# Yelp/nrtsearch

Hardware: AMD Instinct MI355X
Metric: queries/sec, 10M-doc 5-term BM25 top-1000 (higher is better)
Workload: dtype f32

## Files before the change

### nrtsearch_amd/csrc/maxscore.hip

```cpp
#include <hip/hip_runtime.h>
#include <stdint.h>

#include "bm25_common.hiph"

namespace nrtgpu {

constexpr int kMsWinWords = kMsWinDocs / 32;
constexpr int kSl = kMsSlots;
typedef uint32_t u32x2 __attribute__((ext_vector_type(2)));
typedef const NRT_GLOBAL u32x2* gvec2_ptr;

struct alignas(16) WClause {
  uint64_t docids, fnorm;
  uint64_t begin;
  uint32_t count, pad0;
  float    weight;
  int32_t  fx_scale;
  uint32_t flags;
  uint32_t pad;
  uint64_t u_after;
  uint64_t look;
  uint64_t cells, start;
};
static_assert(sizeof(WClause) == 80, "WClause layout");

struct MsSmem {
  uint64_t cand[kMsCandCap];
  uint32_t tab[kTabTerms][kTabEntries];
  float    cache[kLdsCaches][256];
  uint32_t seen[kMsWaves][kMsWinWords];
  WClause  wc[kMsWaves][kMsMaxTerms];
  TopkScratch sc;
  uint64_t theta;
  uint64_t thr;
// ... 175 lines not shown
        __hip_atomic_store(&s.theta, guess, __ATOMIC_RELAXED, __HIP_MEMORY_SCOPE_WORKGROUP);
        __hip_atomic_store(&s.thr, acc_threshold<true>(guess, fx_E), __ATOMIC_RELAXED, __HIP_MEMORY_SCOPE_WORKGROUP);
        atomicMax(theta_g, (unsigned long long)guess);
        atomicMax(s.spec_slot, (unsigned long long)guess);
      }
      s.spec_at = ws >= s.q_wins ? 0u : max(ws * s.spec_grow16 / 16u, ws + (uint32_t)kMsWaves);
      s.n_est += 1u;
    }
  }
  wave_lds_phase();
  if (lane == 0u) __hip_atomic_store(&s.spec_busy, 0u, __ATOMIC_RELEASE, __HIP_MEMORY_SCOPE_WORKGROUP);
}

__device__ __forceinline__ bool ms_reserve(MsSmem& s, uint32_t lane, uint32_t mine, uint32_t& pos) {
  const uint32_t incl = scan64_dpp(mine);
  const uint32_t wave_total = (uint32_t)__builtin_amdgcn_readlane((int)incl, 63);
  uint32_t wbase = 0;
  if (lane == 0) {
    wbase = atomicAdd(&s.cnt, wave_total);
    if (wbase + wave_total > (uint32_t)kMsCandCap) {
      if (wbase <= (uint32_t)kMsCandCap) s.cnt_valid = wbase;
      __hip_atomic_store(&s.rz_flag, 1u, __ATOMIC_RELAXED, __HIP_MEMORY_SCOPE_WORKGROUP);
    }
  }
  wbase = (uint32_t)__builtin_amdgcn_readfirstlane((int)wbase);
  pos = wbase + incl - mine;
  return wbase + wave_total <= (uint32_t)kMsCandCap;
}

template <bool PROF, bool PACKED, int SHAPES>
__global__ __launch_bounds__(kMsThreads)
void bm25_maxscore_kernel(const MsArgs* __restrict__ launch) {
  constexpr bool TWO = SHAPES == 2;
  __shared__ MsSmem s;
  const uint32_t tid = threadIdx.x;
  const uint32_t wave = tid >> 6, lane = tid & 63u;
  for (uint32_t round = 0;; ++round) {
    const uint64_t wall_entry = PROF ? wall_clock64() : 0ull;
    const ms_args_ptr ap = ms_fresh(launch);
    const __attribute__((address_space(4))) DHelp& hp = ap->help;
    const DItem* const items = as_global(ap->items);
    const DPart* const parts = as_global(ap->parts);
    const DWalkRow* const rows = as_global(ap->rows);
  #ifdef NRTGPU_DEV
    const DTerm* const terms = as_global(ap->terms);
  #endif
    const DExchange* const xch = as_global(ap->xch);
    bool helper = false;
    uint32_t my_item = 0, out_slot = 0;
    {
      const uint32_t min_rem = hp.min_rem & 0xFFFFu;
      const bool greedy = ((hp.min_rem >> 16) & 1u) != 0u;
      for (int attempt = 0; attempt < 2; ++attempt) {
        if (tid == 0) {
          s.pick = 0ull;
          s.role[0] = __hip_atomic_load(hp.item_next, __ATOMIC_RELAXED, __HIP_MEMORY_SCOPE_AGENT);
          s.role[1] = __hip_atomic_load(hp.help_used, __ATOMIC_RELAXED, __HIP_MEMORY_SCOPE_AGENT);
          s.role[2] = 0u;
          s.role[3] = __hip_atomic_load(hp.help_off, __ATOMIC_RELAXED, __HIP_MEMORY_SCOPE_AGENT);
        }
        __syncthreads();
        const uint32_t q_next = s.role[0];
        const bool queue_empty = attempt == 1 || q_next >= hp.n_own;
        const bool slots_left = s.role[1] < hp.n_help;
        if (queue_empty && (!slots_left || s.role[3] != 0u)) return;
        const bool look = slots_left && (queue_empty || (hp.alpha16 != 0u && q_next >= hp.n_cus + hp.n_cus / 4u));
// ... 83 lines not shown
    const float tie_breaker = TWO ? q.tie_breaker : 0.0f;
    auto loosen = [&](uint64_t t) { return (TWO && sec_mode == kMsSecReqOpt) ? max(t - (t >> 21), (uint64_t)2) - (uint64_t)1 : t; };
    unsigned int* const my_prune_g = as_global(ap->q_prune) + item.query;
    const uint64_t after_key = q.has_after ? pack_key(q.after_score, (uint32_t)q.after_doc) : ~0ull;

    {
      const uint32_t n_lds = min(item.n_caches, (uint32_t)kLdsCaches) * 256u;
      const float* const caches = as_global(ap->caches);
      for (uint32_t i = tid; i < n_lds; i += kMsThreads) (&s.cache[0][0])[i] = caches[item.cache_off + i];
    }
    for (uint32_t i = tid; i < (uint32_t)kMsCandCap; i += kMsThreads) s.cand[i] = 0ull;
    if (tid == 0) {
      const uint64_t theta0 = __hip_atomic_load(my_theta_g, __ATOMIC_RELAXED, __HIP_MEMORY_SCOPE_AGENT);
      s.theta = theta0;
      s.thr = acc_threshold<true>(theta0, fx_E);
      s.cnt = 0;
      s.cnt_valid = 0;
      s.rz_flag = 0;
      s.spec_busy = 0;
      s.n_meet = s.n_over = s.n_est = 0;
      if (!helper) {
        const unsigned long long now0 = (unsigned long long)wall_clock64();
        __hip_atomic_store(hp.item_t0 + my_item, now0, __ATOMIC_RELAXED, __HIP_MEMORY_SCOPE_AGENT);
        if (my_item == 0u) __hip_atomic_store(hp.t_start, now0, __ATOMIC_RELAXED, __HIP_MEMORY_SCOPE_AGENT);
      }
      s.prune_on = mode == kMsModePrune ? 1u : 0u;
      const bool spec = hp.spec_g != nullptr && hp.spec_z16 != 0u;
      s.wins_started = 0;
      s.q_wins = spec ? as_global(ap->q_wins)[item.query] : 0u;
      s.spec_z16 = spec ? hp.spec_z16 : 0u;
      s.spec_slot = spec ? as_global(hp.spec_g) + item.query : nullptr;
      s.spec_at = spec ? max(hp.spec_sched & 255u, 1u) : 0u;
      s.spec_grow16 = max((hp.spec_sched >> 8) & 255u, 17u);
      s.spec_meet = (hp.spec_sched >> 16) & 1u;
      for (int i = 0; i < kSliceSlots; ++i) s.slot_hits[i] = s.slot_slice[i] = 0u;
      for (int i = 0; i < 16; ++i) s.prof[i] = 0;
    }
    const uint64_t t_item0 = PROF ? __builtin_readcyclecounter() : 0ull;
    const uint64_t wall0 = PROF ? wall_clock64() : 0ull;
    uint64_t tc_meet = 0, tc_part = 0, tc_walk = 0;
    __syncthreads();
    if (xch && tid < 64u) {
      const uint64_t pb = exchange_bound(*xch, item.query, 0ull, tid);
      if (tid == 0 && pb > s.theta) {
        s.theta = pb;
        s.thr = acc_threshold<true>(pb, fx_E);
      }
    }
    for (uint32_t slot = 0; slot < item.n_tabs; ++slot) {
      const float w = items[my_item].tab_weight[slot];
      const int scale = items[my_item].tab_scale[slot];
      const float* cache = &s.cache[items[my_item].tab_cache[slot]][0];
      for (uint32_t e = tid; e < (uint32_t)kTabEntries; e += kMsThreads)
        s.tab[slot][e] = e < (uint32_t)kTabNorms ? 0u : score_value<true>(bm25_score(w, (float)(int32_t)(e >> 7), cache[e & 127u]), scale);
    }
    __syncthreads();
  #ifndef NRT_MS_PHASE_CLOCKS
    if (PROF && tid == 0) s.prof[8] = __builtin_readcyclecounter() - t_item0;
  #endif

    uint32_t* const seen = &s.seen[wave][0];
    WClause* const wcl = &s.wc[wave][0];
    const uint32_t wcl_addr = lds_addr(wcl);
    uint32_t wave_hits = 0;
    uint32_t cur_slot = 0;
    uint64_t pc_post = 0, pc_surv = 0, pc_look = 0, pc_cand = 0, pc_chunks = 0, pc_wins = 0;
  #ifdef NRT_MS_PHASE_CLOCKS
    uint64_t ph[9] = {0, 0, 0, 0, 0, 0, 0, 0, 0}, ph_t = 0;
  #endif
  #ifdef NRT_MS_COUNT_ROUNDS
    uint64_t pc_dense = 0, pc_sparse = 0, pc_steps = 0, pc_tas = 0, pc_crounds = 0;
  #endif
    const uint32_t item_wins = item.flags >> 8;
    uint32_t sc_mul = 1u;
    if (ap->scatter != 0u && item_wins > 3u && item_wins < 65536u) {
      const uint32_t primes[4] = {2654435761u, 2246822519u, 3266489917u, 668265263u};
      uint32_t best = 0xFFFFFFFFu;
  #pragma unroll
      for (int i = 0; i < 4; ++i) {
        const uint32_t a = primes[i] % item_wins;
        const uint32_t x = a * 1000u, y = item_wins * 618u;
        const uint32_t dist = x > y ? x - y : y - x;
        if (a > 1u && dist < best) {
          best = dist;
          sc_mul = a;
        }
      }
    }
    auto window_of_take = [&](uint32_t h) -> uint32_t {
      return (sc_mul == 1u || h >= item_wins) ? h : (h * sc_mul) % item_wins;
    };
    uint32_t g = window_of_take(helper ? (uint32_t)kMsWaves + (uint32_t)__builtin_amdgcn_readfirstlane((int)first_win) : wave);
    uint32_t pi = 0;
    uint32_t win_base = 0;

    const bool parts_by_lane = item.n_parts <= 64u;
    uint32_t part_incl = 0;
    if (parts_by_lane) {
      uint32_t w = 0;
      if (lane < item.n_parts) {
        const u32x2 tr = *(gvec2_ptr)&parts[item.part_begin + lane].tile_begin;
        w = (tr[1] - (tr[0] & ~(win_tiles - 1u)) + win_tiles - 1u) / win_tiles;
      }
      part_incl = scan64_dpp(w);
// ... 105 lines not shown
  #endif
      {
        static_assert(sizeof(DWalkRow) == sizeof(WClause) && sizeof(WClause) % 16 == 0, "a walk row is the image of a WClause");
        const gvec_ptr src = (gvec_ptr)(rows + part.term_begin);
        if (lane < n_terms * (uint32_t)(sizeof(WClause) / 16)) *(u32x4*)lds_ptr(wcl_addr + lane * 16u) = src[lane];
        wave_lds_phase();
        if (lane < n_terms) {
          const uint32_t rec = wcl_addr + lane * (uint32_t)sizeof(WClause);
          my_suf = *(const uint64_t*)lds_ptr(rec + 16u);
          my_flags = *(const uint32_t*)lds_ptr(rec + 40u);
          const u32x4 cs = *(const u32x4*)lds_ptr(rec + 64u);
          my_cells = (gu32_ptr)(((uint64_t)cs[1] << 32) | cs[0]);
          my_start = ((uint64_t)cs[3] << 32) | cs[2];
        }
        my_shift = (my_flags >> 16) & 31u;
      }
      const uint32_t req_mask = TWO ? (uint32_t)__builtin_amdgcn_ballot_w64(lane < n_terms && (my_flags & 8u) != 0u) : 0u;
      const uint32_t first_req = req_mask != 0u ? (uint32_t)__builtin_ctz(req_mask) : 0xFFu;
      if (PROF) tc_part += __builtin_readcyclecounter() - t_part0;

      for (;;) {
        const uint64_t t_win0 = PROF ? __builtin_readcyclecounter() : 0ull;
        const uint32_t ta = (part.tile_begin & ~(win_tiles - 1u)) + (g - win_base) * win_tiles;
        const uint32_t t0 = max(ta, part.tile_begin);
        const uint32_t t1 = min(ta + win_tiles, part.tile_end);
        const uint32_t doc_lo = t0 * (uint32_t)kTileDocs;
        const uint32_t doc_span = min(t1 * (uint32_t)kTileDocs, part.max_doc) - doc_lo;
        if (PROF) pc_wins += 1;
        {
          uint32_t est = 0;
          if (lane == 0) {
            const uint32_t ws = atomicAdd(&s.wins_started, 1u) + 1u, at = s.spec_at;
            if (at != 0u && ws >= at) {
              if (s.spec_meet != 0u) __hip_atomic_store(&s.rz_flag, 1u, __ATOMIC_RELAXED, __HIP_MEMORY_SCOPE_WORKGROUP);
              else est = atomicCAS(&s.spec_busy, 0u, 1u) == 0u ? 1u : 0u;
            }
          }
          if (__builtin_amdgcn_readfirstlane((int)est) != 0)
            ms_estimate((__attribute__((address_space(3))) MsSmem*)&s, k, fx_E, my_theta_g, xch);
        }
        uint32_t g_new = 0;
        if (lane == 0) g_new = (uint32_t)kMsWaves + __hip_atomic_fetch_add(win_next_g, 1u, __ATOMIC_RELAXED, __HIP_MEMORY_SCOPE_AGENT);
        uint64_t theta_other = 0, thr_other = 0;
        if (multi_item) {
          theta_other = __hip_atomic_load(my_theta_g, __ATOMIC_RELAXED, __HIP_MEMORY_SCOPE_AGENT);
          thr_other = acc_threshold<true>(theta_other, fx_E);
          if (mode == kMsModeCount && lane == 0 && __hip_atomic_load(my_prune_g, __ATOMIC_RELAXED, __HIP_MEMORY_SCOPE_AGENT) != 0u)
            __hip_atomic_store(&s.prune_on, 1u, __ATOMIC_RELAXED, __HIP_MEMORY_SCOPE_WORKGROUP);
        }
        uint32_t my_lo = 0, my_hi = 0;
        if (lane < n_terms) {
          my_lo = my_cells[t0 >> my_shift];
          my_hi = my_cells[((t1 - 1u) >> my_shift) + 1u];
        }
        if (n_terms > 1u) {
  #pragma unroll
          for (int j = 0; j < kMsWinWords / 64 / 4; ++j) *(u32x4*)&seen[(lane + 64u * (uint32_t)j) * 4u] = u32x4{0u, 0u, 0u, 0u};
        }
        uint32_t ng = 0;
        {
          const uint64_t thr_w = __hip_atomic_load(&s.prune_on, __ATOMIC_RELAXED, __HIP_MEMORY_SCOPE_WORKGROUP) ? loosen(max(s.thr, thr_other)) : 0ull;
          const uint64_t pb = my_start + my_lo, pe = my_start + my_hi;
          if (lane < n_terms) {
            if (my_suf >= thr_w && pe > pb && (!SHAPES || msm <= 1u || lane + msm <= n_terms) && (!TWO || lane <= first_req)) ng = (uint32_t)((pe - (pb & ~3ull) + (uint64_t)(kSl - 1)) / (uint64_t)kSl);
            *(u32x4*)&wcl[lane].begin = u32x4{(uint32_t)pb, (uint32_t)(pb >> 32), (uint32_t)(pe - pb), 0u};
          }
        }
        const uint32_t incl = scan32_dpp(ng);
        uint32_t pre[kMsMaxTerms];
  #pragma unroll
        for (int i = 0; i < kMsMaxTerms; ++i) pre[i] = (uint32_t)__builtin_amdgcn_readlane((int)incl, i);
        const uint32_t n_groups = pre[kMsMaxTerms - 1];

  #ifdef NRT_MS_PHASE_CLOCKS
        if (PROF) ph_t = t_win0;
  #endif
        NRT_PH_MARK(0);
        for (uint32_t v0 = 0; v0 < n_groups; v0 += 64u) {
          const uint32_t v = v0 + lane;
          const bool act = v < n_groups;
          uint32_t c = 0, before = 0;
  #pragma unroll
          for (int i = 0; i < kMsMaxTerms - 1; ++i) {
            c += (v >= pre[i]) ? 1u : 0u;
            before = (v >= pre[i]) ? pre[i] : before;
          }
          const uint32_t c_first = (uint32_t)__builtin_amdgcn_readfirstlane((int)c);
          const uint64_t theta = max(s.theta, theta_other), thr = loosen(max(s.thr, thr_other));
          const bool pruning = __hip_atomic_load(&s.prune_on, __ATOMIC_RELAXED, __HIP_MEMORY_SCOPE_WORKGROUP) != 0u;
          const uint64_t thr_p = pruning ? thr : 0ull;
          if (readlane_u64(my_suf, c_first) < thr_p) break;
          if (PROF) pc_chunks += 1;
          const uint32_t rec = wcl_addr + c * (uint32_t)sizeof(WClause);
          const u32x4 r0 = *(const u32x4*)lds_ptr(rec), r1 = *(const u32x4*)lds_ptr(rec + 16u), r2 = *(const u32x4*)lds_ptr(rec + 32u);
          const uint64_t u_after = *(const uint64_t*)lds_ptr(rec + 48u);
          const uint64_t col_d = ((uint64_t)r0[1] << 32) | r0[0], col_c = ((uint64_t)r0[3] << 32) | r0[2];
          const uint64_t p_begin = ((uint64_t)r1[1] << 32) | r1[0];
          const uint32_t flags = r2[2];
          const uint32_t q0 = (v - before) * (uint32_t)kSl;
          const uint64_t mine0 = (p_begin & ~3ull) + (uint64_t)q0;
          uint32_t d[kSl], cd[kSl];
  #pragma unroll
          for (int j = 0; j < kSl; ++j) d[j] = cd[j] = 0u;
          if (act) {
            const u32x4 d0 = __builtin_nontemporal_load((gvec_ptr)(col_d + mine0 * 4u));
            const u32x4 d1 = kSl > 4 ? __builtin_nontemporal_load((gvec_ptr)(col_d + mine0 * 4u) + 1) : d0;
            if (PACKED) {
              const uint32_t sw = doc_lo & ~kPackDocMask;
  #pragma unroll
              for (int j = 0; j < 4; ++j) {
                d[j] = (d0[j] >> kPackCodeBits) | sw;
                cd[j] = (d0[j] & kPackCodeMask) << 2;
                if (kSl > 4) {
                  d[(4 + j) % kSl] = (d1[j] >> kPackCodeBits) | sw;
                  cd[(4 + j) % kSl] = (d1[j] & kPackCodeMask) << 2;
                }
              }
            } else {
              const u32x4 c0 = __builtin_nontemporal_load((gvec_ptr)(col_c + mine0 * 4u));
              const u32x4 c1 = kSl > 4 ? __builtin_nontemporal_load((gvec_ptr)(col_c + mine0 * 4u) + 1) : c0;
  #pragma unroll
              for (int j = 0; j < 4; ++j) {
                d[j] = d0[j];
                cd[j] = c0[j];
                if (kSl > 4) {
                  d[(4 + j) % kSl] = d1[j];
                  cd[(4 + j) % kSl] = c1[j];
                }
              }
            }
          }
          NRT_PH_MARK(1);
          uint32_t vmask = 0;
          {
            const uint32_t rel = q0 - ((uint32_t)p_begin & 3u), cnt = act ? r1[2] : 0u;
  #pragma unroll
            for (int j = 0; j < kSl; ++j)
              if (rel + (uint32_t)j < cnt && d[j] - doc_lo < doc_span) vmask |= 1u << j;
          }
          uint32_t val[kSl];
          {
            const uint32_t tab = flags & 7u;
            const char* tb = (const char*)&s.tab[tab == 7u ? 0u : tab][0];
            uint32_t cor = 0;
  #pragma unroll
            for (int j = 0; j < kSl; ++j) {
              val[j] = *(const uint32_t*)(tb + (cd[j] & 0x1FFCu));
              const uint32_t cn = ((vmask >> j) & 1u) ? cd[j] : 0u;
              cor = PACKED ? max(cor, cn) : (cor | cn);
            }
            const bool special = vmask != 0u && ((PACKED ? cor >= (kPackEscBase << 2) : (cor >> 31) != 0u) || tab == 7u);
            if (__any(special)) {
              const float w = __uint_as_float(r2[0]);
              const int fx_scale = (int)r2[1];
              const float* cache = &s.cache[(flags >> 8) & 255u][0];
  #pragma unroll
              for (int j = 0; j < kSl; ++j) {
                uint32_t cj = cd[j];
                if (PACKED && cj >= (kPackEscBase << 2))
                  cj = ((vmask >> j) & 1u) ? packed_escape_word((gu32_ptr)col_c, (uint32_t)mine0 + (uint32_t)j, cj >> 2) : 0x80000100u;
                const bool esc = (cj >> 31) != 0u;
                const uint32_t f = esc ? ((cj >> 8) & 0x3FFFFFu) : ((cj >> 9) & 15u);
                const bool dead = esc ? ((cj >> 30) & 1u) != 0u : (cj >> 20) != 0u;
                const uint32_t nb = esc ? (cj & 255u) : ((cj >> 2) & 127u);
                if (((vmask >> j) & 1u) && (esc || tab == 7u))
                  val[j] = dead ? 0u : score_value<true>(bm25_score(w, (float)(int32_t)f, cache[nb]), fx_scale);
              }
            }
          }
          uint64_t run[kSl];
          uint32_t alive = 0;
          {
            const uint32_t mult = 1u << ((flags >> 4) & 15u);
            uint32_t need_v = 1u;
            if (u_after < thr_p) {
              const uint64_t gap = use_max ? thr_p : thr_p - u_after;
              const uint64_t nv = (gap + (uint64_t)(mult - 1u)) >> ((flags >> 4) & 15u);
              need_v = nv > 0xFFFFFFFFull ? 0xFFFFFFFFu : max((uint32_t)nv, 1u);
            }
            uint32_t pass = 0;
  #pragma unroll
            for (int j = 0; j < kSl; ++j) {
              run[j] = (uint64_t)val[j] * (uint64_t)mult;
              pass |= val[j] >= need_v ? (1u << j) : 0u;
            }
            alive = vmask & pass;
            if (need_v == 0xFFFFFFFFu) {
  #pragma unroll
              for (int j = 0; j < kSl; ++j)
                if ((use_max ? max(run[j], u_after) : run[j] + u_after) < thr_p) alive &= ~(1u << j);
            }
          }
          uint64_t sec[TWO ? kSl : 1];
          if (TWO) {
            if ((req_mask & ((1u << c) - 1u)) != 0u) alive = 0u;
            const bool mine_counts = sec_mode == kMsSecTieBreaker || (sec_mode == kMsSecReqOpt && ((req_mask >> c) & 1u) == 0u);
  #pragma unroll
            for (int j = 0; j < kSl; ++j) sec[j] = mine_counts ? run[j] : 0ull;
          }
          if (PROF) {
            pc_post += (uint64_t)__popc(vmask);
            pc_surv += (uint64_t)__popc(alive);
          }
          NRT_PH_MARK(2);
          const uint32_t c_last = (uint32_t)__builtin_amdgcn_readlane((int)c, (int)(min(n_groups - v0, 64u) - 1u));
          if (n_terms > 1u && __any(alive != 0u)) {
            for (uint32_t cc = c_first; cc <= c_last; ++cc) {
              const uint32_t am = c == cc ? alive : 0u;
              if (!__any(am != 0u)) continue;
  #ifdef NRT_MS_COUNT_ROUNDS
              if (PROF) pc_tas += 1;
  #endif
              uint32_t old[kSl];
  #pragma unroll
              for (int j = 0; j < kSl; ++j) {
                const bool a = (am >> j) & 1u;
                const uint32_t w = a ? ((d[j] - doc_lo) >> 5) : lane;
                old[j] = atomicOr(&seen[w], a ? (1u << (d[j] & 31u)) : 0u);
              }
  #pragma unroll
              for (int j = 0; j < kSl; ++j)
                if (((am >> j) & 1u) && ((old[j] >> (d[j] & 31u)) & 1u)) alive &= ~(1u << j);
            }
          }
          NRT_PH_MARK(3);
          uint32_t ccnt = 0x11111111u;

          for (uint32_t j2 = c_first + 1u; j2 < n_terms; ++j2) {
            if (!__any(alive != 0u)) break;
            const uint64_t S_j = readlane_u64(my_suf, j2);
            uint32_t am = c < j2 ? alive : 0u;
            {
              const uint64_t short_of = S_j < thr_p ? (use_max ? thr_p : thr_p - S_j) : 0ull;
              uint32_t kill = 0;
  #pragma unroll
              for (int j = 0; j < kSl; ++j) kill |= run[j] < short_of ? (1u << j) : 0u;
              if (SHAPES && msm > 1u) {
                const uint32_t left = n_terms - j2;
  #pragma unroll
                for (int j = 0; j < kSl; ++j) kill |= ((ccnt >> (4 * j)) & 15u) + left < msm ? (1u << j) : 0u;
              }
              kill &= am;
              alive &= ~kill;
              am &= ~kill;
            }
            if (!__any(am != 0u)) continue;
            if (PROF) pc_look += (uint64_t)__popc(am);
            const WClause& w2 = wcl[j2];
            const uint64_t look2 = uniform_u64(w2.look);
            const uint32_t flags2 = (uint32_t)__builtin_amdgcn_readfirstlane((int)w2.flags);
            const uint32_t kind2 = (flags2 >> 24) & 7u;
            const uint64_t start2 = uniform_u64(w2.start);
            const gu32_ptr codes2 = (gu32_ptr)(uniform_u64(PACKED ? w2.docids : w2.fnorm) + start2 * 4u);
            uint32_t c2[kSl];
            uint32_t pi2[kSl];
            uint32_t present = 0;
  #ifdef NRT_MS_COUNT_ROUNDS
            if (PROF) { if (kind2 == kLookBits) pc_dense += 1; else pc_sparse += 1; }
  #endif
            if (kind2 == kLookBits) {
              const gvec2_ptr recs = (gvec2_ptr)look2;
              u32x2 r[kSl];
  #pragma unroll
              for (int j = 0; j < kSl; ++j) r[j] = recs[((am >> j) & 1u) ? (d[j] >> 5) : 0u];
              __builtin_amdgcn_sched_barrier(0);
              NRT_PH_MARK(4);
              uint32_t idx[kSl];
  #pragma unroll
              for (int j = 0; j < kSl; ++j) {
                const uint32_t bb = d[j] & 31u;
                const bool there = ((am >> j) & 1u) && ((r[j][0] >> bb) & 1u);
                idx[j] = there ? r[j][1] + (uint32_t)__popc(r[j][0] & ((1u << bb) - 1u)) : 0u;
                present |= (there ? 1u : 0u) << j;
              }
  #pragma unroll
              for (int j = 0; j < kSl; ++j) c2[j] = codes2[idx[j]];
              __builtin_amdgcn_sched_barrier(0);
              NRT_PH_MARK(5);
  #pragma unroll
              for (int j = 0; j < kSl; ++j) pi2[j] = (uint32_t)start2 + idx[j];
            } else {
              const gu32_ptr cells2 = (gu32_ptr)(kind2 == kLookCells ? look2 : uniform_u64(w2.cells));
              const gu32_ptr docs2 = (gu32_ptr)(uniform_u64(w2.docids) + start2 * 4u);
              const uint32_t cshift = kind2 == kLookCells ? (flags2 >> 27) & 31u : 10u + ((flags2 >> 16) & 31u);
              uint32_t a[kSl], b[kSl];
  #pragma unroll
              for (int j = 0; j < kSl; ++j) {
                const uint32_t cell = ((am >> j) & 1u) ? (d[j] >> cshift) : 0u;
                a[j] = cells2[cell];
                b[j] = cells2[cell + 1u];
              }
              uint32_t open = 0;
  #pragma unroll
              for (int j = 0; j < kSl; ++j) {
                if (!((am >> j) & 1u)) b[j] = a[j];
                open |= (a[j] < b[j] ? 1u : 0u) << j;
              }
              while (__any(open != 0u)) {
  #ifdef NRT_MS_COUNT_ROUNDS
                if (PROF) pc_steps += 1;
  #endif
                uint32_t mid[kSl], vv[kSl];
  #pragma unroll
                for (int j = 0; j < kSl; ++j) {
                  mid[j] = (a[j] + b[j]) >> 1;
                  vv[j] = docs2[((open >> j) & 1u) ? mid[j] : 0u];
                }
  #pragma unroll
                for (int j = 0; j < kSl; ++j)
                  if ((open >> j) & 1u) {
                    const uint32_t dv = PACKED ? vv[j] >> kPackCodeBits : vv[j], dd = PACKED ? d[j] & kPackDocMask : d[j];
                    if (dv < dd) a[j] = mid[j] + 1u;
                    else b[j] = mid[j];
                    if (dv == dd) {
                      a[j] = b[j] = mid[j];
                      present |= 1u << j;
                    }
                    if (!(a[j] < b[j])) open &= ~(1u << j);
                  }
              }
  #pragma unroll
              for (int j = 0; j < kSl; ++j) {
                c2[j] = codes2[((present >> j) & 1u) ? a[j] : 0u];
                pi2[j] = (uint32_t)start2 + a[j];
              }
              NRT_PH_MARK(7);
            }
            if (__any(present != 0u)) {
              uint32_t v2[kSl];
              if (PACKED) {
  #pragma unroll
                for (int j = 0; j < kSl; ++j) c2[j] = (c2[j] & kPackCodeMask) << 2;
              }
              values_of_codes<PACKED, kSl>(s, c2, present, flags2 & 7u, w2.weight, w2.fx_scale, (flags2 >> 8) & 255u, w2.fnorm, pi2, v2);
              const uint32_t mult2 = 1u << ((flags2 >> 4) & 15u);
              if (use_max) {
  #pragma unroll
                for (int j = 0; j < kSl; ++j) run[j] = max(run[j], (uint64_t)(((present >> j) & 1u) ? v2[j] : 0u) * (uint64_t)mult2);
              } else if (TWO && sec_mode != kMsSecNone) {
                const bool counts = sec_mode == kMsSecReqOpt && (flags2 & 8u) == 0u;
  #pragma unroll
                for (int j = 0; j < kSl; ++j) {
                  const uint64_t add = (uint64_t)(((present >> j) & 1u) ? v2[j] : 0u) * (uint64_t)mult2;
                  run[j] += add;
                  sec[j] = sec_mode == kMsSecTieBreaker ? max(sec[j], add) : sec[j] + (counts ? add : 0ull);
                }
              } else {
  #pragma unroll
                for (int j = 0; j < kSl; ++j) run[j] += (uint64_t)(((present >> j) & 1u) ? v2[j] : 0u) * (uint64_t)mult2;
              }
              if (SHAPES && msm > 1u) {
                uint32_t x = present;
                x = (x | (x << 12)) & 0x000F000Fu;
                x = (x | (x << 6)) & 0x03030303u;
                x = (x | (x << 3)) & 0x11111111u;
                ccnt += x;
              }
            }
            if (TWO && (flags2 & 8u) != 0u) alive &= ~(am & ~present);
            NRT_PH_MARK(6);
          }

          {
          uint32_t maybe = 0;
  #pragma unroll
          for (int j = 0; j < kSl; ++j)
            if (((alive >> j) & 1u) && run[j] >= thr) maybe |= 1u << j;
          {
            uint32_t pool = pruning ? maybe : alive;
            if (SHAPES && msm > 1u) {
  #pragma unroll
              for (int j = 0; j < kSl; ++j)
                if (((ccnt >> (4 * j)) & 15u) < msm) pool &= ~(1u << j);
            }
            if (part.live_bits != nullptr && __any(pool != 0u)) {
              uint32_t lw[kSl];
  #pragma unroll
              for (int j = 0; j < kSl; ++j) lw[j] = ((const NRT_GLOBAL uint32_t*)part.live_bits)[((pool >> j) & 1u) ? (d[j] >> 5) : 0u];
  #pragma unroll
              for (int j = 0; j < kSl; ++j)
                if (!((lw[j] >> (d[j] & 31u)) & 1u)) pool &= ~(1u << j);
            }
            maybe &= pool;
            uint32_t h = (uint32_t)__popc(pool);
            h = (uint32_t)__builtin_amdgcn_readlane((int)scan64_dpp(h), 63);
            if (mode == kMsModeCount && !pruning) {
              if (lane == 0 && h != 0u) {
                const uint32_t tot = atomicAdd(&s.slot_hits[cur_slot], h) + h;
                if (tot > q.gte_floor) {
                  __hip_atomic_store(&s.prune_on, 1u, __ATOMIC_RELAXED, __HIP_MEMORY_SCOPE_WORKGROUP);
                  if (multi_item) __hip_atomic_store(my_prune_g, 1u, __ATOMIC_RELAXED, __HIP_MEMORY_SCOPE_AGENT);
                }
              }
            } else {
              wave_hits += h;
            }
          }
          uint64_t theta_now = theta;
          while (__any(maybe != 0u)) {
  #ifdef NRT_MS_COUNT_ROUNDS
            if (PROF) pc_crounds += 1;
  #endif
            const uint32_t low = maybe & (0u - maybe);
            uint64_t rsel = run[0], ssel = TWO ? sec[0] : 0ull;
            uint32_t dsel = d[0];
  #pragma unroll
            for (int j = 1; j < kSl; ++j)
              if (low == (1u << j)) {
                rsel = run[j];
                dsel = d[j];
                if (TWO) ssel = sec[j];
              }
            float score = acc_score<true>(rsel, fx_E);
            if (TWO && sec_mode == kMsSecTieBreaker)
              score = (float)(ldexp((double)ssel, -fx_E) + ldexp((double)(rsel - ssel), -fx_E) * (double)tie_breaker);
            else if (TWO && sec_mode == kMsSecReqOpt)
              score = acc_score<true>(rsel - ssel, fx_E) + acc_score<true>(ssel, fx_E);
            const uint64_t key = pack_key(score, (uint32_t)(part.doc_base + (int32_t)dsel));
            const bool want = low != 0u && key > theta_now && key < after_key;
            uint32_t pos = 0;
            if (!__any(want)) {
              maybe &= ~low;
              continue;
            }
            if (ms_reserve(s, lane, want ? 1u : 0u, pos)) {
              if (want) s.cand[pos] = key;
              if (PROF) pc_cand += want ? 1u : 0u;
              maybe &= ~low;
              continue;
            }
            const uint64_t t_m0 = PROF ? __builtin_readcyclecounter() : 0ull;
            (void)ms_meet(s, k, fx_E, my_theta_g, xch, item.query);
            if (PROF) tc_meet += __builtin_readcyclecounter() - t_m0;
            theta_now = max(theta_now, s.theta);
          }
          }
          NRT_PH_MARK(8);
          if (__hip_atomic_load(&s.rz_flag, __ATOMIC_RELAXED, __HIP_MEMORY_SCOPE_WORKGROUP)) {
            const uint64_t t_m0 = PROF ? __builtin_readcyclecounter() : 0ull;
            (void)ms_meet(s, k, fx_E, my_theta_g, xch, item.query);
            if (PROF) tc_meet += __builtin_readcyclecounter() - t_m0;
          }
        }

        if (PROF) tc_walk += __builtin_readcyclecounter() - t_win0;
        g = window_of_take((uint32_t)__builtin_amdgcn_readfirstlane((int)g_new));
        if (g < win_base || g >= win_base + part_wins) break;
      }
    }
    const uint64_t t_idle0 = PROF ? __builtin_readcyclecounter() : 0ull;
    while (ms_meet(s, k, fx_E, my_theta_g, xch, item.query)) {
    }
    const uint64_t t_epi0 = PROF ? __builtin_readcyclecounter() : 0ull;
    if (PROF && lane == 0) {
      atomicAdd((unsigned long long*)&s.prof[10], (unsigned long long)tc_meet);
      atomicAdd((unsigned long long*)&s.prof[11], (unsigned long long)(t_epi0 - t_idle0));
      atomicAdd((unsigned long long*)&s.prof[12], (unsigned long long)tc_part);
      atomicAdd((unsigned long long*)&s.prof[13], (unsigned long long)(tc_walk - tc_meet));
      atomicMax((unsigned long long*)&s.prof[14], (unsigned long long)(t_idle0 - t_item0));
  #ifdef NRT_MS_COUNT_ROUNDS
      atomicAdd((unsigned long long*)&s.prof[11], (unsigned long long)pc_tas - (unsigned long long)(t_epi0 - t_idle0));
      atomicAdd((unsigned long long*)&s.prof[12], (unsigned long long)pc_dense - (unsigned long long)tc_part);
      atomicAdd((unsigned long long*)&s.prof[10], (unsigned long long)pc_sparse - (unsigned long long)tc_meet);
      atomicAdd((unsigned long long*)&s.prof[13], (unsigned long long)pc_steps - (unsigned long long)(tc_walk - tc_meet));
      atomicAdd((unsigned long long*)&s.prof[8], (unsigned long long)pc_crounds);
  #endif
    }

    {
      const uint32_t c = s.cnt;
      __syncthreads();
      if (c > k) {
        uint64_t thr = 0;
        const uint32_t m = topk_compact<kMsThreads, kMsCandCap>(s.cand, c, k, &s.sc, &thr);
        if (tid == 0) s.cnt = m;
      }
    }
    if (lane == 0 && wave_hits) atomicAdd(&s.slot_hits[cur_slot], wave_hits);
  #ifdef NRT_MS_PHASE_CLOCKS
    if (PROF && lane == 0) {
  #pragma unroll
      for (int i = 0; i < 9; ++i) atomicAdd((unsigned long long*)&s.prof[i], (unsigned long long)ph[i]);
    }
    if (false) {
  #else
    if (PROF && lane == 0) {
      atomicAdd((unsigned long long*)&s.prof[0], (unsigned long long)pc_wins);
      atomicAdd((unsigned long long*)&s.prof[2], (unsigned long long)pc_chunks);
    }
    if (PROF) {
  #endif
      uint64_t v3 = pc_post, v4 = pc_surv, v6 = pc_look, v7 = pc_cand;
  #pragma unroll
// ... 234 lines not shown
```

### nrtsearch_amd/csrc/search.cpp

```cpp
#include "runtime_internal.h"


static uint32_t spec_margin16(const nrtgpu_ctx* ctx) { return (uint32_t)std::max(ctx->spec_z16.load(std::memory_order_relaxed), 0); }
static void spec_sync_epoch(const nrtgpu_ctx* ctx, LeafSetCache* lsc) {
  const uint64_t e = ctx->spec_epoch.load(std::memory_order_relaxed);
  if (lsc->spec_epoch.exchange(e, std::memory_order_relaxed) != e) {
    lsc->spec_queries.store(0, std::memory_order_relaxed);
    lsc->spec_reruns.store(0, std::memory_order_relaxed);
    lsc->spec_calls.store(0, std::memory_order_relaxed);
    lsc->spec_calls_rerun.store(0, std::memory_order_relaxed);
    lsc->spec_scattered.store(0, std::memory_order_relaxed);
    lsc->spec_off.store(0, std::memory_order_relaxed);
  }
}
static bool speculating(nrtgpu_ctx* ctx, const nrtgpu_seg* const* segs, int32_t n_segs) {
  if (!ctx || spec_margin16(ctx) == 0u || !segs || n_segs <= 0) return false;
  for (int32_t i = 0; i < n_segs; ++i)
    if (!segs[i]) return false;
  std::shared_ptr<LeafSetCache> lsc = leaf_set_cache(ctx, segs, n_segs);
  spec_sync_epoch(ctx, lsc.get());
  return lsc->spec_off.load(std::memory_order_relaxed) == 0;
}
static void note_speculation_of(nrtgpu_ctx* ctx, LeafSetCache* lsc, int64_t n_queries, int64_t n_rerun) {
  spec_sync_epoch(ctx, lsc);
// ... 98 lines not shown
  help.win_next = (uint32_t*)(wb + L.hwin);
  help.help_cnt = (uint32_t*)(wb + L.hcnt);
  help.item_t0 = (unsigned long long*)(wb + L.ht0);
  help.help_head = (uint32_t*)(wb + L.hhead);
  help.help_query = (uint32_t*)(wb + L.hnext);
  help.help_off = (uint32_t*)(wb + L.hoff);
  help.item_next = (uint32_t*)(wb + L.hqueue);
  help.help_used = (uint32_t*)(wb + L.hused);
  help.t_start = (unsigned long long*)(wb + L.hstart);
  {
    static const int env_help_alpha = (int)dev_env_int("NRTGPU_MS_HELP_ALPHA", 24);
    uint64_t wins = 0;
    for (size_t i = 0; i < hp.n_ms_items; ++i) wins += hp.items[i].flags >> 8;
    help.total_wins = (uint32_t)std::min<uint64_t>(wins, 0xFFFFFFFFull);
    help.alpha16 = (uint32_t)std::max(env_help_alpha, 0);
    static const int env_spare = (int)dev_env_int("NRTGPU_MS_SPARE_CUS", 8);
    help.n_cus = (uint32_t)std::max(ctx->n_cus - std::max(env_spare, 0), 1);
    if (small) help.n_cus = (uint32_t)std::max(env_spare, 1);
    help.persistent = ms_persistent() ? 1u : 0u;
  }
  help.n_own = (uint32_t)hp.n_ms_items;
  help.n_help = (uint32_t)L.n_help;
  help.slot_base = (uint32_t)L.n_items;
  static const int env_help_min = (int)dev_env_int("NRTGPU_MS_HELP_MIN", 16);
  static const bool env_help_greedy = dev_env_int("NRTGPU_MS_HELP_GREEDY", 0) != 0;
  help.min_rem = (uint32_t)std::min(std::max(env_help_min, 1), 0xFFFF) | (env_help_greedy ? 1u << 16 : 0u);
  help.walls = L.profile ? (unsigned long long*)(wb + L.walls) : nullptr;
  help.spec_g = L.spec ? (unsigned long long*)(wb + L.spec_g) : nullptr;
  help.spec_z16 = L.spec ? L.spec_z16 : 0u;
  {
    const int env_first = (int)dev_env_int("NRTGPU_MS_SPEC_FIRST", 2 * kMsWaves);
    const int env_grow = (int)dev_env_int("NRTGPU_MS_SPEC_GROW", 32);
    const bool env_meet = dev_env_int("NRTGPU_MS_SPEC_MEET", 0) != 0;
    help.spec_sched = (uint32_t)std::min(std::max(env_first, 1), 255) | ((uint32_t)std::min(std::max(env_grow, 17), 255) << 8) | (env_meet ? 1u << 16 : 0u);
  }
  MsArgs ms_args{};
  ms_args.items = (const DItem*)(db + L.items);
  ms_args.parts = (const DPart*)(db + L.parts);
  ms_args.terms = (const DTerm*)(wb + L.terms);
  ms_args.queries = (const DQuery*)(db + L.queries);
  ms_args.caches = (const float*)(db + L.caches);
  ms_args.theta_g = (unsigned long long*)(db + L.theta);
  ms_args.slice_sum = (uint32_t*)(wb + L.ssum);
  ms_args.q_prune = (uint32_t*)(wb + L.qprune);
  ms_args.xch = L.use_xch ? (const DExchange*)(db + L.xch) : nullptr;
  ms_args.item_keys = (uint64_t*)(wb + L.item_keys);
  ms_args.item_counts = (uint32_t*)(wb + L.item_counts);
  ms_args.item_hits = (uint64_t*)(wb + L.item_hits);
  ms_args.item_prof = L.profile ? (uint64_t*)(wb + L.prof) : nullptr;
  ms_args.q_wins = (const uint32_t*)(db + L.q_wins);
  ms_args.rows = L.walk_rows ? (const DWalkRow*)(wb + L.rows) : nullptr;
  {
    const long forced = dev_env_int("NRTGPU_MS_SCATTER", -1);
    ms_args.scatter = forced >= 0 ? (forced != 0 ? 1u : 0u) : ((L.spec && hp.lsc->spec_scattered.load(std::memory_order_relaxed) != 0) ? 1u : 0u);
  }
  ms_args.k_stride = hp.k_stride;
  ms_args.help = help;
  return ms_args;
}

static int enqueue_search(nrtgpu_ctx* ctx, Slot* slot, const HostPlan& hp, int32_t n_queries, uint32_t k_stride_out, const SearchOpts& o,
                          DeviceRun* run, std::unique_lock<std::mutex>& gpu) {
  forget_foreign_hip_error();
  static const bool follow_up_on = dev_env_int("NRTGPU_FOLLOW_UP", 1) != 0;
  const bool small = o.follow_up && follow_up_on && hp.n_ms_items != 0 && hp.n_ms_items == hp.items.size() && ms_persistent();
  const SearchLayout L(ctx, hp, n_queries, k_stride_out, o, ms_helpers(ctx, hp));
  const size_t n_items = L.n_items, n_help = L.n_help, n_ms = hp.n_ms_items;
// ... 947 lines not shown
```

Baseline: 557,100.

## Split eight-posting units across lane pairs when a window has few groups

The walk loop body becomes a templated lambda. When a window's remaining group count is 32 or less (and slots per unit is eight), each unit is split across two lanes that take four postings each, instead of one lane taking eight. This uses idle lanes, roughly halves per-lane serial work and register pressure in the gather and lookup chains, and keeps more memory requests in flight. The cost is a second instantiation of a large body, which raises code size and compile time. The path can be disabled by an environment variable, but only in DEV builds.

```diff
diff --git a/nrtsearch_amd/csrc/maxscore.hip b/nrtsearch_amd/csrc/maxscore.hip
--- a/nrtsearch_amd/csrc/maxscore.hip
+++ b/nrtsearch_amd/csrc/maxscore.hip
@@ -1,5 +1,7 @@
 #include <hip/hip_runtime.h>
 #include <stdint.h>
+
+#include <type_traits>
 
 #include "bm25_common.hiph"
 
@@ -241,6 +243,7 @@
 __global__ __launch_bounds__(kMsThreads)
 void bm25_maxscore_kernel(const MsArgs* __restrict__ launch) {
   constexpr bool TWO = SHAPES == 2;
+  constexpr bool kMsHalfBody = kSl == 8;
   __shared__ MsSmem s;
   const uint32_t tid = threadIdx.x;
   const uint32_t wave = tid >> 6, lane = tid & 63u;
@@ -390,7 +393,7 @@
       s.spec_slot = spec ? as_global(hp.spec_g) + item.query : nullptr;
       s.spec_at = spec ? max(hp.spec_sched & 255u, 1u) : 0u;
       s.spec_grow16 = max((hp.spec_sched >> 8) & 255u, 17u);
-      s.spec_meet = (hp.spec_sched >> 16) & 1u;
+      s.spec_meet = (hp.spec_sched >> 16) & 3u;
       for (int i = 0; i < kSliceSlots; ++i) s.slot_hits[i] = s.slot_slice[i] = 0u;
       for (int i = 0; i < 16; ++i) s.prof[i] = 0;
     }
@@ -427,7 +430,7 @@
     uint64_t ph[9] = {0, 0, 0, 0, 0, 0, 0, 0, 0}, ph_t = 0;
   #endif
   #ifdef NRT_MS_COUNT_ROUNDS
-    uint64_t pc_dense = 0, pc_sparse = 0, pc_steps = 0, pc_tas = 0, pc_crounds = 0;
+    uint64_t pc_dense = 0, pc_sparse = 0, pc_steps = 0, pc_tas = 0, pc_crounds = 0, pc_half = 0, pc_half_rounds = 0;
   #endif
     const uint32_t item_wins = item.flags >> 8;
     uint32_t sc_mul = 1u;
@@ -599,7 +602,7 @@
           if (lane == 0) {
             const uint32_t ws = atomicAdd(&s.wins_started, 1u) + 1u, at = s.spec_at;
             if (at != 0u && ws >= at) {
-              if (s.spec_meet != 0u) __hip_atomic_store(&s.rz_flag, 1u, __ATOMIC_RELAXED, __HIP_MEMORY_SCOPE_WORKGROUP);
+              if ((s.spec_meet & 1u) != 0u) __hip_atomic_store(&s.rz_flag, 1u, __ATOMIC_RELAXED, __HIP_MEMORY_SCOPE_WORKGROUP);
               else est = atomicCAS(&s.spec_busy, 0u, 1u) == 0u ? 1u : 0u;
             }
           }
@@ -638,14 +641,23 @@
   #pragma unroll
         for (int i = 0; i < kMsMaxTerms; ++i) pre[i] = (uint32_t)__builtin_amdgcn_readlane((int)incl, i);
         const uint32_t n_groups = pre[kMsMaxTerms - 1];
+  #ifdef NRTGPU_DEV
+        const bool half_on = (__builtin_amdgcn_readfirstlane((int)s.spec_meet) & 2) == 0;
+  #else
+        constexpr bool half_on = true;
+  #endif
 
   #ifdef NRT_MS_PHASE_CLOCKS
         if (PROF) ph_t = t_win0;
   #endif
         NRT_PH_MARK(0);
-        for (uint32_t v0 = 0; v0 < n_groups; v0 += 64u) {
-          const uint32_t v = v0 + lane;
-          const bool act = v < n_groups;
+        auto walk_units = [&](auto ns_c, auto half_c, const uint32_t v0) __attribute__((always_inline)) -> bool {
+          constexpr int NS = decltype(ns_c)::value;
+          constexpr bool HALF = decltype(half_c)::value;
+          static_assert(!HALF || (NS == 4 && kSl == 8), "the half body: four of a unit's eight postings per lane");
+          const uint32_t n_lanes = HALF ? 2u * (n_groups - v0) : min(n_groups - v0, 64u);
+          const uint32_t v = HALF ? v0 + (lane >> 1) : v0 + lane;
+          const bool act = HALF ? lane < n_lanes : v < n_groups;
           uint32_t c = 0, before = 0;
   #pragma unroll
           for (int i = 0; i < kMsMaxTerms - 1; ++i) {
@@ -656,7 +668,7 @@
           const uint64_t theta = max(s.theta, theta_other), thr = loosen(max(s.thr, thr_other));
           const bool pruning = __hip_atomic_load(&s.prune_on, __ATOMIC_RELAXED, __HIP_MEMORY_SCOPE_WORKGROUP) != 0u;
           const uint64_t thr_p = pruning ? thr : 0ull;
-          if (readlane_u64(my_suf, c_first) < thr_p) break;
+          if (readlane_u64(my_suf, c_first) < thr_p) return false;
           if (PROF) pc_chunks += 1;
           const uint32_t rec = wcl_addr + c * (uint32_t)sizeof(WClause);
           const u32x4 r0 = *(const u32x4*)lds_ptr(rec), r1 = *(const u32x4*)lds_ptr(rec + 16u), r2 = *(const u32x4*)lds_ptr(rec + 32u);
@@ -664,35 +676,35 @@
           const uint64_t col_d = ((uint64_t)r0[1] << 32) | r0[0], col_c = ((uint64_t)r0[3] << 32) | r0[2];
           const uint64_t p_begin = ((uint64_t)r1[1] << 32) | r1[0];
           const uint32_t flags = r2[2];
-          const uint32_t q0 = (v - before) * (uint32_t)kSl;
+          const uint32_t q0 = (v - before) * (uint32_t)kSl + (HALF ? (lane & 1u) * 4u : 0u);
           const uint64_t mine0 = (p_begin & ~3ull) + (uint64_t)q0;
-          uint32_t d[kSl], cd[kSl];
-  #pragma unroll
-          for (int j = 0; j < kSl; ++j) d[j] = cd[j] = 0u;
+          uint32_t d[NS], cd[NS];
+  #pragma unroll
+          for (int j = 0; j < NS; ++j) d[j] = cd[j] = 0u;
           if (act) {
             const u32x4 d0 = __builtin_nontemporal_load((gvec_ptr)(col_d + mine0 * 4u));
-            const u32x4 d1 = kSl > 4 ? __builtin_nontemporal_load((gvec_ptr)(col_d + mine0 * 4u) + 1) : d0;
+            const u32x4 d1 = NS > 4 ? __builtin_nontemporal_load((gvec_ptr)(col_d + mine0 * 4u) + 1) : d0;
             if (PACKED) {
               const uint32_t sw = doc_lo & ~kPackDocMask;
   #pragma unroll
               for (int j = 0; j < 4; ++j) {
                 d[j] = (d0[j] >> kPackCodeBits) | sw;
                 cd[j] = (d0[j] & kPackCodeMask) << 2;
-                if (kSl > 4) {
-                  d[(4 + j) % kSl] = (d1[j] >> kPackCodeBits) | sw;
-                  cd[(4 + j) % kSl] = (d1[j] & kPackCodeMask) << 2;
+                if (NS > 4) {
+                  d[(4 + j) % NS] = (d1[j] >> kPackCodeBits) | sw;
+                  cd[(4 + j) % NS] = (d1[j] & kPackCodeMask) << 2;
                 }
               }
             } else {
               const u32x4 c0 = __builtin_nontemporal_load((gvec_ptr)(col_c + mine0 * 4u));
-              const u32x4 c1 = kSl > 4 ? __builtin_nontemporal_load((gvec_ptr)(col_c + mine0 * 4u) + 1) : c0;
+              const u32x4 c1 = NS > 4 ? __builtin_nontemporal_load((gvec_ptr)(col_c + mine0 * 4u) + 1) : c0;
   #pragma unroll
               for (int j = 0; j < 4; ++j) {
                 d[j] = d0[j];
                 cd[j] = c0[j];
-                if (kSl > 4) {
-                  d[(4 + j) % kSl] = d1[j];
-                  cd[(4 + j) % kSl] = c1[j];
+                if (NS > 4) {
+                  d[(4 + j) % NS] = d1[j];
+                  cd[(4 + j) % NS] = c1[j];
                 }
               }
             }
@@ -702,16 +714,16 @@
           {
             const uint32_t rel = q0 - ((uint32_t)p_begin & 3u), cnt = act ? r1[2] : 0u;
   #pragma unroll
-            for (int j = 0; j < kSl; ++j)
+            for (int j = 0; j < NS; ++j)
               if (rel + (uint32_t)j < cnt && d[j] - doc_lo < doc_span) vmask |= 1u << j;
           }
-          uint32_t val[kSl];
+          uint32_t val[NS];
           {
             const uint32_t tab = flags & 7u;
             const char* tb = (const char*)&s.tab[tab == 7u ? 0u : tab][0];
             uint32_t cor = 0;
   #pragma unroll
-            for (int j = 0; j < kSl; ++j) {
+            for (int j = 0; j < NS; ++j) {
               val[j] = *(const uint32_t*)(tb + (cd[j] & 0x1FFCu));
               const uint32_t cn = ((vmask >> j) & 1u) ? cd[j] : 0u;
               cor = PACKED ? max(cor, cn) : (cor | cn);
@@ -722,7 +734,7 @@
               const int fx_scale = (int)r2[1];
               const float* cache = &s.cache[(flags >> 8) & 255u][0];
   #pragma unroll
-              for (int j = 0; j < kSl; ++j) {
+              for (int j = 0; j < NS; ++j) {
                 uint32_t cj = cd[j];
                 if (PACKED && cj >= (kPackEscBase << 2))
                   cj = ((vmask >> j) & 1u) ? packed_escape_word((gu32_ptr)col_c, (uint32_t)mine0 + (uint32_t)j, cj >> 2) : 0x80000100u;
@@ -735,7 +747,7 @@
               }
             }
           }
-          uint64_t run[kSl];
+          uint64_t run[NS];
           uint32_t alive = 0;
           {
             const uint32_t mult = 1u << ((flags >> 4) & 15u);
@@ -747,30 +759,30 @@
             }
             uint32_t pass = 0;
   #pragma unroll
-            for (int j = 0; j < kSl; ++j) {
+            for (int j = 0; j < NS; ++j) {
               run[j] = (uint64_t)val[j] * (uint64_t)mult;
               pass |= val[j] >= need_v ? (1u << j) : 0u;
             }
             alive = vmask & pass;
             if (need_v == 0xFFFFFFFFu) {
   #pragma unroll
-              for (int j = 0; j < kSl; ++j)
+              for (int j = 0; j < NS; ++j)
                 if ((use_max ? max(run[j], u_after) : run[j] + u_after) < thr_p) alive &= ~(1u << j);
             }
           }
-          uint64_t sec[TWO ? kSl : 1];
+          uint64_t sec[TWO ? NS : 1];
           if (TWO) {
             if ((req_mask & ((1u << c) - 1u)) != 0u) alive = 0u;
             const bool mine_counts = sec_mode == kMsSecTieBreaker || (sec_mode == kMsSecReqOpt && ((req_mask >> c) & 1u) == 0u);
   #pragma unroll
-            for (int j = 0; j < kSl; ++j) sec[j] = mine_counts ? run[j] : 0ull;
+            for (int j = 0; j < NS; ++j) sec[j] = mine_counts ? run[j] : 0ull;
           }
           if (PROF) {
             pc_post += (uint64_t)__popc(vmask);
             pc_surv += (uint64_t)__popc(alive);
           }
           NRT_PH_MARK(2);
-          const uint32_t c_last = (uint32_t)__builtin_amdgcn_readlane((int)c, (int)(min(n_groups - v0, 64u) - 1u));
+          const uint32_t c_last = (uint32_t)__builtin_amdgcn_readlane((int)c, (int)(n_lanes - 1u));
           if (n_terms > 1u && __any(alive != 0u)) {
             for (uint32_t cc = c_first; cc <= c_last; ++cc) {
               const uint32_t am = c == cc ? alive : 0u;
@@ -778,15 +790,15 @@
   #ifdef NRT_MS_COUNT_ROUNDS
               if (PROF) pc_tas += 1;
   #endif
-              uint32_t old[kSl];
-  #pragma unroll
-              for (int j = 0; j < kSl; ++j) {
+              uint32_t old[NS];
+  #pragma unroll
+              for (int j = 0; j < NS; ++j) {
                 const bool a = (am >> j) & 1u;
                 const uint32_t w = a ? ((d[j] - doc_lo) >> 5) : lane;
                 old[j] = atomicOr(&seen[w], a ? (1u << (d[j] & 31u)) : 0u);
               }
   #pragma unroll
-              for (int j = 0; j < kSl; ++j)
+              for (int j = 0; j < NS; ++j)
                 if (((am >> j) & 1u) && ((old[j] >> (d[j] & 31u)) & 1u)) alive &= ~(1u << j);
             }
           }
@@ -801,11 +813,11 @@
               const uint64_t short_of = S_j < thr_p ? (use_max ? thr_p : thr_p - S_j) : 0ull;
               uint32_t kill = 0;
   #pragma unroll
-              for (int j = 0; j < kSl; ++j) kill |= run[j] < short_of ? (1u << j) : 0u;
+              for (int j = 0; j < NS; ++j) kill |= run[j] < short_of ? (1u << j) : 0u;
               if (SHAPES && msm > 1u) {
                 const uint32_t left = n_terms - j2;
   #pragma unroll
-                for (int j = 0; j < kSl; ++j) kill |= ((ccnt >> (4 * j)) & 15u) + left < msm ? (1u << j) : 0u;
+                for (int j = 0; j < NS; ++j) kill |= ((ccnt >> (4 * j)) & 15u) + left < msm ? (1u << j) : 0u;
               }
               kill &= am;
               alive &= ~kill;
@@ -819,47 +831,47 @@
             const uint32_t kind2 = (flags2 >> 24) & 7u;
             const uint64_t start2 = uniform_u64(w2.start);
             const gu32_ptr codes2 = (gu32_ptr)(uniform_u64(PACKED ? w2.docids : w2.fnorm) + start2 * 4u);
-            uint32_t c2[kSl];
-            uint32_t pi2[kSl];
+            uint32_t c2[NS];
+            uint32_t pi2[NS];
             uint32_t present = 0;
   #ifdef NRT_MS_COUNT_ROUNDS
             if (PROF) { if (kind2 == kLookBits) pc_dense += 1; else pc_sparse += 1; }
   #endif
             if (kind2 == kLookBits) {
               const gvec2_ptr recs = (gvec2_ptr)look2;
-              u32x2 r[kSl];
-  #pragma unroll
-              for (int j = 0; j < kSl; ++j) r[j] = recs[((am >> j) & 1u) ? (d[j] >> 5) : 0u];
+              u32x2 r[NS];
+  #pragma unroll
+              for (int j = 0; j < NS; ++j) r[j] = recs[((am >> j) & 1u) ? (d[j] >> 5) : 0u];
               __builtin_amdgcn_sched_barrier(0);
               NRT_PH_MARK(4);
-              uint32_t idx[kSl];
-  #pragma unroll
-              for (int j = 0; j < kSl; ++j) {
+              uint32_t idx[NS];
+  #pragma unroll
+              for (int j = 0; j < NS; ++j) {
                 const uint32_t bb = d[j] & 31u;
                 const bool there = ((am >> j) & 1u) && ((r[j][0] >> bb) & 1u);
                 idx[j] = there ? r[j][1] + (uint32_t)__popc(r[j][0] & ((1u << bb) - 1u)) : 0u;
                 present |= (there ? 1u : 0u) << j;
               }
   #pragma unroll
-              for (int j = 0; j < kSl; ++j) c2[j] = codes2[idx[j]];
+              for (int j = 0; j < NS; ++j) c2[j] = codes2[idx[j]];
               __builtin_amdgcn_sched_barrier(0);
               NRT_PH_MARK(5);
   #pragma unroll
-              for (int j = 0; j < kSl; ++j) pi2[j] = (uint32_t)start2 + idx[j];
+              for (int j = 0; j < NS; ++j) pi2[j] = (uint32_t)start2 + idx[j];
             } else {
               const gu32_ptr cells2 = (gu32_ptr)(kind2 == kLookCells ? look2 : uniform_u64(w2.cells));
               const gu32_ptr docs2 = (gu32_ptr)(uniform_u64(w2.docids) + start2 * 4u);
               const uint32_t cshift = kind2 == kLookCells ? (flags2 >> 27) & 31u : 10u + ((flags2 >> 16) & 31u);
-              uint32_t a[kSl], b[kSl];
-  #pragma unroll
-              for (int j = 0; j < kSl; ++j) {
+              uint32_t a[NS], b[NS];
+  #pragma unroll
+              for (int j = 0; j < NS; ++j) {
                 const uint32_t cell = ((am >> j) & 1u) ? (d[j] >> cshift) : 0u;
                 a[j] = cells2[cell];
                 b[j] = cells2[cell + 1u];
               }
               uint32_t open = 0;
   #pragma unroll
-              for (int j = 0; j < kSl; ++j) {
+              for (int j = 0; j < NS; ++j) {
                 if (!((am >> j) & 1u)) b[j] = a[j];
                 open |= (a[j] < b[j] ? 1u : 0u) << j;
               }
@@ -867,14 +879,14 @@
   #ifdef NRT_MS_COUNT_ROUNDS
                 if (PROF) pc_steps += 1;
   #endif
-                uint32_t mid[kSl], vv[kSl];
-  #pragma unroll
-                for (int j = 0; j < kSl; ++j) {
+                uint32_t mid[NS], vv[NS];
+  #pragma unroll
+                for (int j = 0; j < NS; ++j) {
                   mid[j] = (a[j] + b[j]) >> 1;
                   vv[j] = docs2[((open >> j) & 1u) ? mid[j] : 0u];
                 }
   #pragma unroll
-                for (int j = 0; j < kSl; ++j)
+                for (int j = 0; j < NS; ++j)
                   if ((open >> j) & 1u) {
                     const uint32_t dv = PACKED ? vv[j] >> kPackCodeBits : vv[j], dd = PACKED ? d[j] & kPackDocMask : d[j];
                     if (dv < dd) a[j] = mid[j] + 1u;
@@ -887,34 +899,34 @@
                   }
               }
   #pragma unroll
-              for (int j = 0; j < kSl; ++j) {
+              for (int j = 0; j < NS; ++j) {
                 c2[j] = codes2[((present >> j) & 1u) ? a[j] : 0u];
                 pi2[j] = (uint32_t)start2 + a[j];
               }
               NRT_PH_MARK(7);
             }
             if (__any(present != 0u)) {
-              uint32_t v2[kSl];
+              uint32_t v2[NS];
               if (PACKED) {
   #pragma unroll
-                for (int j = 0; j < kSl; ++j) c2[j] = (c2[j] & kPackCodeMask) << 2;
-              }
-              values_of_codes<PACKED, kSl>(s, c2, present, flags2 & 7u, w2.weight, w2.fx_scale, (flags2 >> 8) & 255u, w2.fnorm, pi2, v2);
+                for (int j = 0; j < NS; ++j) c2[j] = (c2[j] & kPackCodeMask) << 2;
+              }
+              values_of_codes<PACKED, NS>(s, c2, present, flags2 & 7u, w2.weight, w2.fx_scale, (flags2 >> 8) & 255u, w2.fnorm, pi2, v2);
               const uint32_t mult2 = 1u << ((flags2 >> 4) & 15u);
               if (use_max) {
   #pragma unroll
-                for (int j = 0; j < kSl; ++j) run[j] = max(run[j], (uint64_t)(((present >> j) & 1u) ? v2[j] : 0u) * (uint64_t)mult2);
+                for (int j = 0; j < NS; ++j) run[j] = max(run[j], (uint64_t)(((present >> j) & 1u) ? v2[j] : 0u) * (uint64_t)mult2);
               } else if (TWO && sec_mode != kMsSecNone) {
                 const bool counts = sec_mode == kMsSecReqOpt && (flags2 & 8u) == 0u;
   #pragma unroll
-                for (int j = 0; j < kSl; ++j) {
+                for (int j = 0; j < NS; ++j) {
                   const uint64_t add = (uint64_t)(((present >> j) & 1u) ? v2[j] : 0u) * (uint64_t)mult2;
                   run[j] += add;
                   sec[j] = sec_mode == kMsSecTieBreaker ? max(sec[j], add) : sec[j] + (counts ? add : 0ull);
                 }
               } else {
   #pragma unroll
-                for (int j = 0; j < kSl; ++j) run[j] += (uint64_t)(((present >> j) & 1u) ? v2[j] : 0u) * (uint64_t)mult2;
+                for (int j = 0; j < NS; ++j) run[j] += (uint64_t)(((present >> j) & 1u) ? v2[j] : 0u) * (uint64_t)mult2;
               }
               if (SHAPES && msm > 1u) {
                 uint32_t x = present;
@@ -931,21 +943,21 @@
           {
           uint32_t maybe = 0;
   #pragma unroll
-          for (int j = 0; j < kSl; ++j)
+          for (int j = 0; j < NS; ++j)
             if (((alive >> j) & 1u) && run[j] >= thr) maybe |= 1u << j;
           {
             uint32_t pool = pruning ? maybe : alive;
             if (SHAPES && msm > 1u) {
   #pragma unroll
-              for (int j = 0; j < kSl; ++j)
+              for (int j = 0; j < NS; ++j)
                 if (((ccnt >> (4 * j)) & 15u) < msm) pool &= ~(1u << j);
             }
             if (part.live_bits != nullptr && __any(pool != 0u)) {
-              uint32_t lw[kSl];
-  #pragma unroll
-              for (int j = 0; j < kSl; ++j) lw[j] = ((const NRT_GLOBAL uint32_t*)part.live_bits)[((pool >> j) & 1u) ? (d[j] >> 5) : 0u];
-  #pragma unroll
-              for (int j = 0; j < kSl; ++j)
+              uint32_t lw[NS];
+  #pragma unroll
+              for (int j = 0; j < NS; ++j) lw[j] = ((const NRT_GLOBAL uint32_t*)part.live_bits)[((pool >> j) & 1u) ? (d[j] >> 5) : 0u];
+  #pragma unroll
+              for (int j = 0; j < NS; ++j)
                 if (!((lw[j] >> (d[j] & 31u)) & 1u)) pool &= ~(1u << j);
             }
             maybe &= pool;
@@ -972,7 +984,7 @@
             uint64_t rsel = run[0], ssel = TWO ? sec[0] : 0ull;
             uint32_t dsel = d[0];
   #pragma unroll
-            for (int j = 1; j < kSl; ++j)
+            for (int j = 1; j < NS; ++j)
               if (low == (1u << j)) {
                 rsel = run[j];
                 dsel = d[j];
@@ -1003,6 +1015,26 @@
           }
           }
           NRT_PH_MARK(8);
+          return true;
+        };
+        for (uint32_t v0 = 0; v0 < n_groups; v0 += 64u) {
+          bool more;
+          if (kMsHalfBody && n_groups - v0 <= 32u && half_on) {
+  #ifdef NRT_MS_COUNT_ROUNDS
+            const uint64_t chunks0 = pc_chunks, look0 = pc_dense + pc_sparse;
+  #endif
+            if constexpr (kMsHalfBody) more = walk_units(std::integral_constant<int, 4>{}, std::true_type{}, v0);
+            else more = false;
+  #ifdef NRT_MS_COUNT_ROUNDS
+            if (PROF) {
+              pc_half += pc_chunks - chunks0;
+              pc_half_rounds += pc_dense + pc_sparse - look0;
+            }
+  #endif
+          } else {
+            more = walk_units(std::integral_constant<int, kSl>{}, std::false_type{}, v0);
+          }
+          if (!more) break;
           if (__hip_atomic_load(&s.rz_flag, __ATOMIC_RELAXED, __HIP_MEMORY_SCOPE_WORKGROUP)) {
             const uint64_t t_m0 = PROF ? __builtin_readcyclecounter() : 0ull;
             (void)ms_meet(s, k, fx_E, my_theta_g, xch, item.query);
@@ -1024,8 +1056,10 @@
       atomicAdd((unsigned long long*)&s.prof[11], (unsigned long long)(t_epi0 - t_idle0));
       atomicAdd((unsigned long long*)&s.prof[12], (unsigned long long)tc_part);
       atomicAdd((unsigned long long*)&s.prof[13], (unsigned long long)(tc_walk - tc_meet));
+  #ifndef NRT_MS_COUNT_ROUNDS
       atomicMax((unsigned long long*)&s.prof[14], (unsigned long long)(t_idle0 - t_item0));
-  #ifdef NRT_MS_COUNT_ROUNDS
+  #else
+      atomicAdd((unsigned long long*)&s.prof[14], (unsigned long long)pc_half | ((unsigned long long)pc_half_rounds << 32));
       atomicAdd((unsigned long long*)&s.prof[11], (unsigned long long)pc_tas - (unsigned long long)(t_epi0 - t_idle0));
       atomicAdd((unsigned long long*)&s.prof[12], (unsigned long long)pc_dense - (unsigned long long)tc_part);
       atomicAdd((unsigned long long*)&s.prof[10], (unsigned long long)pc_sparse - (unsigned long long)tc_meet);
diff --git a/nrtsearch_amd/csrc/search.cpp b/nrtsearch_amd/csrc/search.cpp
--- a/nrtsearch_amd/csrc/search.cpp
+++ b/nrtsearch_amd/csrc/search.cpp
@@ -154,7 +154,9 @@
     const int env_first = (int)dev_env_int("NRTGPU_MS_SPEC_FIRST", 2 * kMsWaves);
     const int env_grow = (int)dev_env_int("NRTGPU_MS_SPEC_GROW", 32);
     const bool env_meet = dev_env_int("NRTGPU_MS_SPEC_MEET", 0) != 0;
-    help.spec_sched = (uint32_t)std::min(std::max(env_first, 1), 255) | ((uint32_t)std::min(std::max(env_grow, 17), 255) << 8) | (env_meet ? 1u << 16 : 0u);
+    const bool env_half = dev_env_int("NRTGPU_MS_HALF_GROUPS", 1) != 0;
+    help.spec_sched = (uint32_t)std::min(std::max(env_first, 1), 255) | ((uint32_t)std::min(std::max(env_grow, 17), 255) << 8) | (env_meet ? 1u << 16 : 0u) |
+                      (env_half ? 0u : 1u << 17);
   }
   MsArgs ms_args{};
   ms_args.items = (const DItem*)(db + L.items);
```

Result: faster. 563,600 (median of 6 runs) (+1.2%).
